# JiYuanFeng/DDP

Hardware: AMD Instinct MI355X
Metric: images/s at K DDIM steps (512x1024, 150-class) per GPU and whole node (higher is better)
Workload: dtype f32 (bf16x3-split MFMA products, fp32 accumulate); 1 GPU; ade_swin_t_k3_8x512x1024 (ADE20K Swin-T DDP decode head, 3-step DDIM, batch 8x512x1024 per GPU; x (8,256,128,256), random-init weights); images_per_call=8, ddim_steps=3, parallelism=dp1 (independent images, weights broadcast once), gemm_engine=bf16x3

## Files before the change

ddp_amd/_lib.py:

```python
import ctypes as C
import os

from . import build as _build

MAX_LAYERS = 12
MAX_STEPS = 64
ABI_VERSION = 6

TASK_SEG, TASK_DEPTH, TASK_BEV = 0, 1, 2
SAMPLER_DDIM, SAMPLER_DDPM = 0, 1
GEMM_F32_MFMA, GEMM_BF16X3 = 0, 1
FLAG_UNFUSED_LAYER, FLAG_UNFUSED_PROLOGUE, FLAG_RECORD_X0, FLAG_GATHER_GUESS_ZERO, FLAG_FCN_PREPARED, FLAG_FORCE_X0, FLAG_UNFUSED_TAIL, FLAG_SB_HEAD = 1, 2, 4, 8, 16, 32, 64, 128
FLAG_DEPTH_SCALE_UP, FLAG_DEPTH_NO_EPS = 256, 512
DEPTH_NORM_LINEAR, DEPTH_NORM_SOFTMAX, DEPTH_NORM_SIGMOID = 0, 1, 2
MAX_DEPTH_BINS = 256
NECK_WEIGHTS_READY = 1

_fp = C.c_void_p


class DdpCfg(C.Structure):
    _fields_ = [
        ('abi_version', C.c_int32), ('task', C.c_int32), ('sampler', C.c_int32), ('batch', C.c_int32),
        ('randsteps', C.c_int32), ('timesteps', C.c_int32), ('num_layers', C.c_int32),
# ... 3 lines not shown
        ('threshold', C.c_float),
        ('bev_in_min', C.c_float * 2), ('bev_in_max', C.c_float * 2),
        ('bev_out_first', C.c_float * 2), ('bev_out_step', C.c_float * 2),
        ('gemm_mode', C.c_int32), ('flags', C.c_int32),
        ('depth_n_bins', C.c_int32), ('depth_norm', C.c_int32), ('head_min_depth', C.c_float), ('head_max_depth', C.c_float),
    ]


LAYER_FIELDS = ['sampling_offsets_w', 'sampling_offsets_b', 'attention_weights_w', 'attention_weights_b',
                'value_proj_w', 'value_proj_b', 'output_proj_w', 'output_proj_b', 'ffn0_w', 'ffn0_b',
                'ffn1_w', 'ffn1_b', 'norm0_w', 'norm0_b', 'norm1_w', 'norm1_b', 'time_w', 'time_b']


class DdpLayerWeights(C.Structure):
    _fields_ = [(n, _fp) for n in LAYER_FIELDS]


TOP_FIELDS = ['transform_w', 'transform_b', 'time_freq', 'time1_w', 'time1_b', 'time3_w', 'time3_b',
              'embedding', 'head_w', 'head_b']


class DdpWeights(C.Structure):
    _fields_ = [(n, _fp) for n in TOP_FIELDS] + [('layers', DdpLayerWeights * MAX_LAYERS), ('depth_bins', _fp)]


class DdpStep(C.Structure):
    _fields_ = [('time_in', C.c_float), ('alpha', C.c_float), ('sigma', C.c_float),
                ('alpha_next', C.c_float), ('sigma_next', C.c_float), ('ddpm_c', C.c_float),
                ('ddpm_std', C.c_float), ('ddpm_add_noise', C.c_int32)]


class DdpFpnLevel(C.Structure):
    _fields_ = [('lat_w', _fp), ('lat_gn_w', _fp), ('lat_gn_b', _fp), ('out_w', _fp), ('out_gn_w', _fp), ('out_gn_b', _fp),
                ('in_channels', C.c_int), ('h', C.c_int), ('w', C.c_int)]


class DdpFcnConv(C.Structure):
    _fields_ = [('conv_w', _fp), ('conv_b', _fp), ('bn_w', _fp), ('bn_b', _fp), ('bn_mean', _fp), ('bn_var', _fp),
                ('bn_eps', C.c_float), ('time_w', _fp), ('time_b', _fp)]


class DdpSegAug(C.Structure):
    _fields_ = [('d_scores', _fp), ('h', C.c_int32), ('w', C.c_int32), ('img_h', C.c_int32), ('img_w', C.c_int32),
                ('crop_h', C.c_int32), ('crop_w', C.c_int32), ('flip', C.c_int32)]


class DdpDepthAug(C.Structure):
    _fields_ = [('d_depth', _fp), ('h', C.c_int32), ('w', C.c_int32), ('flip', C.c_int32)]


MAX_AUGS = 16
MAX_WINDOWS = 64

EXPORTS = ['ddp_last_error', 'ddp_abi_version', 'ddp_query_workspace', 'ddp_query_const_workspace', 'ddp_prepare',
           'ddp_prepare_geometry', 'ddp_sample', 'ddp_msda_forward_lds_workspace', 'ddp_msda_forward_lds', 'ddp_seg_aug_postprocess', 'ddp_seg_slide_postprocess', 'ddp_depth_postprocess',
           'ddp_x0_trace', 'ddp_head_forward', 'ddp_msda_forward', 'ddp_linear', 'ddp_linear_b3_workspace', 'ddp_linear_b3', 'ddp_time_embed', 'ddp_ddim_update_seg',
           'ddp_seg_x0_project', 'ddp_seg_postprocess', 'ddp_neck_msm_workspace', 'ddp_neck_msm', 'ddp_fcn_head_workspace', 'ddp_fcn_head_forward', 'ddp_sample_fcn_workspace', 'ddp_prepare_fcn', 'ddp_sample_fcn', 'ddp_neck_fpn_workspace', 'ddp_neck_fpn', 'ddp_neck_fpn_msm_workspace', 'ddp_neck_fpn_msm', 'ddp_profile_begin', 'ddp_profile_end', 'ddp_profile_read']

_libs = {}


class DdpError(RuntimeError):
    pass


def lib_path():
    return os.environ.get('DDP_LIB_PATH') or _build.LIB_PATH


def load(path=None):
    path = os.path.abspath(path or lib_path())
    if path in _libs:
        return _libs[path]
    if not os.path.exists(path):
        raise DdpError(f'{path} not found: build it with `python -m ddp_amd.build` '
                       '(hipcc --offload-arch=gfx950); ddp_amd has no non-HIP fallback')
    if path == os.path.abspath(_build.LIB_PATH) and _build.built_hash() != _build.source_hash():
        raise DdpError(f'{path} is stale: built from sources {_build.built_hash() or "<no stamp>"}, the tree holds '
                       f'{_build.source_hash()}; rebuild with `python -m ddp_amd.build`')
    lib = C.CDLL(path)
    lib.ddp_last_error.restype = C.c_char_p
    lib.ddp_abi_version.restype = C.c_int
    lib.ddp_query_workspace.argtypes = [C.POINTER(DdpCfg), C.POINTER(C.c_size_t)]
    lib.ddp_prepare.argtypes = [C.POINTER(DdpCfg), C.POINTER(DdpWeights), C.POINTER(DdpStep), _fp, _fp]
    lib.ddp_query_const_workspace.argtypes = [C.POINTER(DdpCfg), C.POINTER(C.c_size_t)]
    lib.ddp_prepare_geometry.argtypes = [C.POINTER(DdpCfg), _fp, _fp]
    lib.ddp_msda_forward_lds_workspace.argtypes = [C.c_int, C.c_int, C.c_int, C.POINTER(C.c_size_t)]
    lib.ddp_msda_forward_lds.argtypes = [_fp, _fp, _fp, _fp, C.c_int, C.c_int, C.c_int, _fp, _fp]
    lib.ddp_seg_aug_postprocess.argtypes = [C.POINTER(DdpSegAug), C.c_int, C.c_int, C.c_int, C.c_int, C.c_int, C.c_int, _fp, _fp,
                                            _fp]
    lib.ddp_seg_slide_postprocess.argtypes = [C.POINTER(_fp), C.POINTER(C.c_int), C.POINTER(C.c_int)] + [C.c_int] * 17 + [_fp, _fp, _fp]
    lib.ddp_depth_postprocess.argtypes = [C.POINTER(DdpDepthAug), C.c_int, C.c_int, C.c_int, C.c_int, C.c_int, C.c_float, C.c_float,
                                          _fp, _fp]
    lib.ddp_sample.argtypes = [C.POINTER(DdpCfg), C.POINTER(DdpWeights), C.POINTER(DdpStep), _fp, _fp, _fp, _fp,
                               _fp, _fp]
    lib.ddp_x0_trace.argtypes = [C.POINTER(DdpCfg), _fp, C.POINTER(C.c_void_p)]
    lib.ddp_head_forward.argtypes = [C.POINTER(DdpCfg), C.POINTER(DdpWeights), _fp, _fp, _fp, _fp, _fp]
    lib.ddp_msda_forward.argtypes = [_fp, _fp, _fp, C.c_int, C.c_int, C.c_int, _fp]
    lib.ddp_linear.argtypes = [_fp, _fp, _fp, _fp, C.c_int, C.c_int, C.c_int, C.c_int, _fp]
    lib.ddp_linear_b3_workspace.argtypes = [C.c_int, C.c_int, C.c_int, C.POINTER(C.c_size_t)]
    lib.ddp_linear_b3.argtypes = [_fp, _fp, _fp, _fp, C.c_int, C.c_int, C.c_int, _fp, _fp]
    lib.ddp_time_embed.argtypes = [C.POINTER(DdpWeights), C.c_int, C.POINTER(C.c_float), C.c_int, _fp, _fp, _fp, _fp]
    lib.ddp_ddim_update_seg.argtypes = [_fp, C.c_int, C.c_int, _fp, _fp, C.c_int, C.POINTER(DdpStep), _fp]
    lib.ddp_seg_x0_project.argtypes = [_fp, C.c_int, C.c_int, C.c_int, _fp, C.c_float, _fp, _fp]
    lib.ddp_seg_postprocess.argtypes = [_fp] + [C.c_int] * 12 + [_fp, _fp]
    lib.ddp_neck_msm_workspace.argtypes = [C.c_int, C.POINTER(C.c_int), C.POINTER(C.c_int), C.POINTER(C.c_size_t)]
    lib.ddp_neck_msm.argtypes = [C.POINTER(_fp), C.POINTER(C.c_int), C.POINTER(C.c_int), C.c_int, _fp, _fp, _fp, C.c_int, C.c_int, _fp,
# ... 30 lines not shown
```

ddp_amd/csrc/ddp_api.hip:

```cpp
#include <stdarg.h>
#include <stdio.h>
#include <string.h>

#include <initializer_list>

#include "ddp_internal.h"

namespace ddp {

static thread_local char g_err[512] = "";

void set_error(const char* fmt, ...) {
  va_list ap;
  va_start(ap, fmt);
  vsnprintf(g_err, sizeof(g_err), fmt, ap);
  va_end(ap);
}

int check_launch(const char* what) {
  hipError_t e = hipGetLastError();
  if (e != hipSuccess) {
    set_error("%s: %s", what, hipGetErrorString(e));
    return DDP_E_LAUNCH;
  }
// ... 456 lines not shown
      return DDP_E_LAUNCH;
    }
    DDP_TRY(launch_pack_conv3x3_scaled(w->head_w, nullptr, o.bins_wpack, o.nbins, 256, st));
    if (o.b3) {
      DDP_TRY(launch_split_weights(o.bins_wpack, 2304, 256, 2304, o.bins_wsplit, st));
      DDP_TRY(launch_build_stages(o.bins_wsplit, size_t(256) * 2304, 2304, 256, 0, 1, 72, 0, 2, 1, 0, o.bins_stream, st));
    }
  }
  for (int l = 0; l < o.L; ++l) {
    const ddp_layer_weights& lw = w->layers[l];
    DDP_TRY(launch_pack_rows(lw.sampling_offsets_w, 64, lw.attention_weights_w, 32, o.wcat[l], 256, st));
    DDP_TRY(launch_pack_rows(lw.sampling_offsets_b, 64, lw.attention_weights_b, 32, o.bcat[l], 1, st));
  }
  if (o.b3) {
    auto wr = [](const SplitW& w) { return const_cast<unsigned short*>(w.p); };
    DDP_TRY(launch_split_weights(o.wx, o.Cx, 256, o.Cx, wr(o.wp_x), st));
    if (c->task != DDP_TASK_DEPTH) DDP_TRY(launch_split_weights(o.wm, 256, 256, 256, wr(o.wp_m), st));
    if (c->task == DDP_TASK_DEPTH) DDP_TRY(launch_split_weights(o.wtap, 256, 9, 256, wr(o.wp_head), st));
    else DDP_TRY(launch_split_weights(w->head_w, 256, o.Kc, 256, wr(o.wp_head), st));
    for (int l = 0; l < o.L; ++l) {
      const ddp_layer_weights& lw = w->layers[l];
      DDP_TRY(launch_split_weights(lw.value_proj_w, 256, 256, 256, wr(o.wp_v[l]), st));
      DDP_TRY(launch_split_weights(o.wcat[l], 256, 96, 256, wr(o.wp_cat[l]), st));
      DDP_TRY(launch_split_weights(lw.output_proj_w, 256, 256, 256, wr(o.wp_o[l]), st));
      DDP_TRY(launch_split_weights(lw.ffn0_w, 256, DDP_FFN, 256, wr(o.wp_f0[l]), st));
      DDP_TRY(launch_split_weights(lw.ffn1_w, DDP_FFN, 256, DDP_FFN, wr(o.wp_f1[l]), st));
    }
    if (c->task == DDP_TASK_SEG) {
      const int nch = (o.Kc + 63) / 64;
      DDP_TRY(launch_build_stages(o.wp_head.p, o.wp_head.comp_stride, 256, o.Kc, 1, nch, 2, 0, 0, 1, 2, o.tail_stream, st));
      DDP_TRY(bias_table(o.tail_bias, {{0, w->head_b, o.Kc}}, "seg tail", st));
      DDP_TRY(launch_build_stages(o.wp_head.p, o.wp_head.comp_stride, 256, o.Kc, 1, nch, 2, 0, 0, 1, 2, o.tail4_stream, st));
      DDP_TRY(build_proj_images(o, 0, o.tail4_stream, 2 * nch, st));
      DDP_TRY(bias_table(o.tail4_bias, {{0, w->head_b, o.Kc}, {DDP_FFN, w->layers[0].value_proj_b, 256}}, "fused tail", st));
      DDP_TRY(launch_linear(o.lut, 256, false, o.wm, 256, nullptr, nullptr, 0, 0, 0, o.tlut, 256, o.Kc + 1, 256, 256, 0, st));
    }
    if (c->task != DDP_TASK_DEPTH)
      DDP_TRY(launch_build_stages(o.wp_m.p, o.wp_m.comp_stride, 256, 256, 0, 1, 8, 0, 2, 1, 0, o.pro_stream, st));
    DDP_TRY(build_proj_images(o, 0, o.pro_stream, 8, st));
    DDP_TRY(bias_table(o.pro_bias, {{DDP_FFN, w->layers[0].value_proj_b, 256}}, "prologue", st));
    if (o.head7_stream) {
      DDP_TRY(launch_build_stages(o.wp_m.p, o.wp_m.comp_stride, 256, 256, 0, 1, 8, 0, 2, 1, 0, o.head7_stream, st));
      DDP_TRY(launch_build_stages(o.wp_x.p, o.wp_x.comp_stride, 256, 256, 0, 1, 8, 8, 2, 1, 0, o.head7_stream, st));
      if (hipMemcpyAsync(o.head7_stream + size_t(16) * 48 * 1024, o.pro_stream + size_t(8) * 48 * 1024, size_t(11) * 48 * 1024,
                         hipMemcpyDeviceToDevice, st) != hipSuccess) {
        set_error("first-step head stream copy failed");
        return DDP_E_LAUNCH;
      }
    }
    for (int l = 0; l < o.L; ++l) {
      const ddp_layer_weights& lw = w->layers[l];
      unsigned char* sp = o.wstream[l];
      DDP_TRY(launch_build_stages(o.wp_o[l].p, o.wp_o[l].comp_stride, 256, 256, 0, 1, 8, 0, 2, 1, 0, sp, st));
      DDP_TRY(launch_build_stages(o.wp_f0[l].p, o.wp_f0[l].comp_stride, 256, DDP_FFN, 1, 16, 2, 8, 0, 1, 4, sp, st));
      DDP_TRY(launch_build_stages(o.wp_f1[l].p, o.wp_f1[l].comp_stride, DDP_FFN, 256, 0, 1, 32, 10, 4, 1, 0, sp, st));
      DDP_TRY(bias_table(o.bias_ext[l], {{0, lw.ffn0_b, DDP_FFN}}, "layer", st));
      if (l + 1 < o.L) {
        DDP_TRY(build_proj_images(o, l + 1, sp, 72, st));
        if (hipMemcpyAsync(o.bias_ext[l] + DDP_FFN, w->layers[l + 1].value_proj_b, 256 * sizeof(float), hipMemcpyDeviceToDevice, st) !=
            hipSuccess) {
          set_error("bias table copy failed");
          return DDP_E_LAUNCH;
        }
      }
    }
    if (o.lt_stream && c->task != DDP_TASK_SEG) {
      const size_t sb = size_t(48) * 1024;
      const int rows = c->task == DDP_TASK_DEPTH ? 9 : o.Kc;
      DDP_TRY(launch_build_stages(o.wp_head.p, o.wp_head.comp_stride, 256, rows, 1, 1, 2, 0, 0, 1, 2, o.tail_stream, st));
      DDP_TRY(bias_table(o.tail_bias, {{0, c->task == DDP_TASK_BEV ? w->head_b : nullptr, o.Kc}}, "head tail", st));
      if (hipMemcpyAsync(o.lt_stream, o.wstream[o.L - 1], 72 * sb, hipMemcpyDeviceToDevice, st) != hipSuccess ||
          hipMemcpyAsync(o.lt_stream + 72 * sb, o.tail_stream, 2 * sb, hipMemcpyDeviceToDevice, st) != hipSuccess) {
        set_error("layer + tail stream copy failed");
        return DDP_E_LAUNCH;
      }
      DDP_TRY(bias_table(o.lt_bias, {{0, w->layers[o.L - 1].ffn0_b, DDP_FFN}}, "layer + tail", st));
    }
    if (o.wvs) {
      DDP_TRY(launch_matvec(w->layers[0].value_proj_w, nullptr, o.wm, o.wvs, 256, 256, 1, 256, 256, 0, 0, st));
      DDP_TRY(launch_matvec(o.wcat[0], nullptr, o.wm, o.wvs + 256, 256, 96, 1, 256, 96, 0, 0, st));
    }
    if (o.lut64) {
      DDP_TRY(launch_build_bev_lut(w->embedding, o.lut64, o.Kc, c->bit_scale, st));
      DDP_TRY(launch_linear(o.lut64, 256, false, o.wm, 256, nullptr, nullptr, 0, 0, 0, o.tlut, 256, 1 << o.Kc, 256, 256, 0, st));
    }
    if (o.lt_stream && c->task == DDP_TASK_SEG) {
      const int nch = (o.Kc + 63) / 64;
      const size_t sb = size_t(48) * 1024;
      if (hipMemcpyAsync(o.lt_stream, o.wstream[o.L - 1], 72 * sb, hipMemcpyDeviceToDevice, st) != hipSuccess ||
          hipMemcpyAsync(o.lt_stream + 72 * sb, o.tail4_stream, size_t(2 * nch + 11) * sb, hipMemcpyDeviceToDevice, st) != hipSuccess) {
        set_error("layer + tail stream copy failed");
        return DDP_E_LAUNCH;
      }
      DDP_TRY(bias_table(o.lt_bias, {{0, w->layers[o.L - 1].ffn0_b, DDP_FFN}, {DDP_FFN, w->layers[0].value_proj_b, 256}}, "layer + tail",
                         st));
    }
  }
  return DDP_OK;
}

int publish_q(const Layout& o, const float* row_major, hipStream_t st) {
  if (o.b3 && !o.fused_layer) return launch_row_to_sb(row_major, 256, o.q_sb, int(o.M), 256, st);
  return launch_row_to_blk(row_major, o.q, int(o.M), st);
}

int depth_bins_head(const ddp_cfg* c, const Layout& o, float* pred, hipStream_t st) {
  const int M = int(o.M);
  DepthBinsArgs a;
// ... 417 lines not shown
    DDP_TRY(launch_bev_resample(o.xproj, o.s, o.B, geom, st));
    DDP_TRY(launch_nchw_to_sb(d_noise, o.in_sb, o.R, 256, o.N, st));
    DDP_TRY(launch_b3_linear(o.in_sb, o.wp_m, nullptr, nullptr, 0, 0, 0, o.feat0, 256, M0, 256, 256, st, TAG_FEAT));
  } else {
    DDP_TRY(launch_nchw_to_tok(d_noise, o.mask, o.R, 256, o.N, st));
  }
  TailLaunch tl{};
  tl.Q = o.q;
  tl.M = int(o.M);
  tl.num_classes = o.Kc;
  tl.kind = 1;
  tl.prob = o.prob;
  tl.threshold = c->threshold;
  tl.x0_idx = code;
  tl.ldl = 32;
  for (int s = 0; s < o.K; ++s) {
    const ddp_step& sp = steps[s];
    const float* aff = o.aff + size_t(s) * o.L * 512;
    if (p.bev_chain) {
      if (s > 0) {
        const ddp_step& pp = steps[s - 1];
        const float ua = pp.sigma_next / (pp.sigma > 1e-8f ? pp.sigma : 1e-8f);
        DDP_TRY(launch_bev_u_update(o.feat0, code, o.tlut, o.R, geom, ua, pp.alpha_next - pp.alpha * ua, st));
      }
      DDP_TRY(launch_bev_q(o.feat0, o.s, o.q, o.R, o.r, geom, st));
    } else {
      if (o.b3) {
        DDP_TRY(launch_row_to_sb(o.mask, 256, o.in_sb, M0, 256, st));
        DDP_TRY(launch_b3_linear(o.in_sb, o.wp_m, nullptr, o.xproj, 256, o.r * o.N, o.N, o.feat0, 256, M0, 256, 256, st, TAG_XPROJ));
      } else {
        DDP_TRY(launch_linear(o.mask, 256, false, o.wm, 256, nullptr, o.xproj, 256, o.r * o.N, o.N, o.feat0, 256, M0, 256, 256, 0, st));
      }
      DDP_TRY(launch_bev_resample(o.feat0, o.s, o.R, geom, st));
      DDP_TRY(publish_q(o, o.s, st));
    }
    tl.prob_mode = s == 0 ? 1 : 2;
    DDP_TRY(encoder_forward(w, o, aff, st, false, !p.bev_chain, p.bev_chain ? &tl : nullptr));
    if (p.bev_chain) continue;
    DDP_TRY(head_gemm(c, w, o, st));
    DDP_TRY(launch_bev_update(bev_update_args(c, w, o, o.mask, s == 0, sp), st));
  }
  return launch_finalize_nchw(o.prob, 32, d_out, o.B, o.r, o.Nh, o.Kc, float(o.r * o.K), st);
}

}
}

using namespace ddp;

extern "C" {

const char* ddp_last_error(void) { return g_err; }
int ddp_abi_version(void) { return DDP_ABI_VERSION; }

int ddp_profile_begin(int tag) {
  if ((tag < 0 || tag >= TAG_COUNT) && tag != PROF_ALL) {
    set_error("profile: unknown tag %d", tag);
    return DDP_E_BADCFG;
  }
  if (!g_prof.created) {
    for (int i = 0; i < 2 * PROF_MAX; ++i)
      if (hipEventCreate(&g_prof.ev[i]) != hipSuccess) {
        set_error("hipEventCreate failed");
        return DDP_E_LAUNCH;
      }
    g_prof.created = true;
  }
  g_prof.n = 0;
  g_prof.tag = tag;
  g_prof.resolved = false;
  return DDP_OK;
}

int ddp_profile_end(float* total_ms, int* launches) {
  const int n = g_prof.n;
  g_prof.tag = -1;
  float tot = 0.f;
  for (int i = 0; i < n; ++i) {
    if (hipEventSynchronize(g_prof.ev[2 * i + 1]) != hipSuccess) {
      set_error("hipEventSynchronize failed");
      return DDP_E_LAUNCH;
    }
    float ms = 0.f;
    (void)hipEventElapsedTime(&ms, g_prof.ev[2 * i], g_prof.ev[2 * i + 1]);
    g_prof.ms[i] = ms;
    tot += ms;
  }
  g_prof.resolved = true;
  if (total_ms) *total_ms = tot;
  if (launches) *launches = n;
  return DDP_OK;
}

int ddp_profile_read(int tag, float* total_ms, int* launches) {
  if (tag < 0 || tag >= TAG_COUNT) {
    set_error("profile: unknown tag %d", tag);
    return DDP_E_BADCFG;
  }
  if (!g_prof.resolved) {
    set_error("profile: no finished session (call ddp_profile_end first)");
    return DDP_E_BADCFG;
  }
  float tot = 0.f;
  int cnt = 0;
  for (int i = 0; i < g_prof.n; ++i)
    if (g_prof.rec_tag[i] == tag) {
// ... 1093 lines not shown
```

ddp_amd/csrc/ddp_internal.h:

```cpp
#pragma once
#include <hip/hip_runtime.h>
#include <stddef.h>
#include <atomic>
#include "../../include/ddp_mi355x.h"


#ifndef DDP_S_F32
#define DDP_S_F32 1
#endif

namespace ddp {

void set_error(const char* fmt, ...);
int check_launch(const char* what);

struct LdsAttrOnce {
  std::atomic<unsigned long long> done{0};
  void ensure(const void* fn, int bytes) {
    int dev = 0;
    (void)hipGetDevice(&dev);
    if (dev >= 0 && dev < 64 && ((done.load(std::memory_order_acquire) >> dev) & 1ull)) return;
    if (hipFuncSetAttribute(fn, hipFuncAttributeMaxDynamicSharedMemorySize, bytes) != hipSuccess) {
      (void)hipGetLastError();
      set_error("hipFuncSetAttribute(MaxDynamicSharedMemorySize = %d) failed on device %d", bytes, dev);
// ... 1 lines not shown
    }
    if (dev >= 0 && dev < 64) done.fetch_or(1ull << dev, std::memory_order_release);
  }
};
inline int cu_count() {
  static std::atomic<int> cache[64];
  int dev = 0;
  (void)hipGetDevice(&dev);
  if (dev >= 0 && dev < 64) {
    const int c = cache[dev].load(std::memory_order_relaxed);
    if (c > 0) return c;
  }
  int n = 0;
  if (hipDeviceGetAttribute(&n, hipDeviceAttributeMultiprocessorCount, dev) != hipSuccess || n <= 0) n = 256;
  if (dev >= 0 && dev < 64) cache[dev].store(n, std::memory_order_relaxed);
  return n;
}

enum GemmTag {
  TAG_GENERIC = 0, TAG_XPROJ = 1, TAG_FEAT = 2, TAG_VALUE = 3, TAG_SAMP = 4, TAG_OUTPROJ_LN = 5, TAG_FC1 = 6,
  TAG_FC2_LN = 7, TAG_HEAD = 8, TAG_GATHER = 9, TAG_LAYER_TAIL = 10, TAG_COUNT = 11
};
void prof_begin(int tag, hipStream_t st);
void prof_end(int tag, hipStream_t st);

int launch_linear(const float* A, int lda, bool a_blk, const float* W, int ldw, const float* bias, const float* add,
                  int ld_add, int rn, int n_tok, float* out, int ldo, int M, int N, int K, int gelu, hipStream_t st,
                  int tag = TAG_GENERIC);
int launch_linear_blk(const float* A, int lda, bool a_blk, const float* W, int ldw, const float* bias,
                      const float* add, int ld_add, int rn, int n_tok, float* out_blk, int M, int N, int K, int gelu,
                      hipStream_t st);
int launch_linear_res_ln_blk(const float* A, int lda, bool a_blk, const float* W, int ldw, const float* bias,
                             const float* res_blk, const float* ga_aff, const float* be_aff, float* out_blk, int M,
                             int K, hipStream_t st);
int launch_linear_samp(const float* A_blk, const float* Wcat, const float* py, const float* px, int n_tok, int w,
                       float* out, int M, hipStream_t st);

struct SplitW {
  const unsigned short* p;
  size_t comp_stride;
};
int launch_b3_linear(const unsigned short* A_sb, const SplitW& w, const float* bias, const float* add, int ld_add,
                     int rn, int n_tok, float* out, int ldo, int M, int N, int K, hipStream_t st, int tag);
int launch_b3_linear_sb(const unsigned short* A_sb, const SplitW& w, const float* bias, const float* add, int ld_add,
                        int rn, int n_tok, unsigned short* out_sb, float* out_f32_blk, int M, int N, int K, int gelu,
                        hipStream_t st, int tag);
int launch_b3_linear_res_ln(const unsigned short* A_sb, const SplitW& w, const float* bias, const float* res_blk,
                            const unsigned short* res_sb, const float* ga_aff, const float* be_aff, float* out_f32_blk,
                            unsigned short* out_sb, int M, int K, hipStream_t st, int tag);
int launch_b3_linear_samp(const unsigned short* A_sb, const SplitW& wcat, const float* py, const float* px, int n_tok,
                          int w, float* out, int M, hipStream_t st);
int launch_build_stages(const unsigned short* Wp, size_t comp_stride, int K, int rows_valid, int tall, int n_rowblk, int n_kblk,
                        int base, int a, int b, int c, unsigned char* stream, hipStream_t st);
struct LayerLaunch {
  const unsigned short* S;
  const float* Sf;
  float* Q;
  unsigned short* Q_sb;
  const unsigned char* stream;
  const float* bias_ext;
  const float *bo, *ga0, *be0, *b2, *ga1, *be1;
  int M, has_next;
  float* v_out;
  float* samp_out;
  const float *py, *px;
  int n_tok, w;
  const float* res_f;
  const float* wm;
  const float* dvec;
};
int launch_b3_layer(const LayerLaunch& a, hipStream_t st);
struct TailLaunch {
  float* Q;
  const unsigned char* stream;
  const float* bias_ext;
  const float* lut;
  float* prob;
  unsigned short* mask_sb;
  unsigned char* x0_idx;
  const unsigned char* x0_force;
  int M, num_classes, ldl, prob_mode;
  float alpha, sigma, alpha_next, sigma_next;
  int fuse_next;
  float* ubuf;
  const float* tlut;
  const float* res;
  int res_rn;
  int res_frag;
  float* v_out;
  float* samp_out;
  const float *py, *px;
  int n_tok, w;
  int kind;
  float threshold;
};
int launch_b3_tail(const TailLaunch& a, hipStream_t st);
bool b3_layer_tail_supported(int num_classes);
int launch_b3_layer_tail(const LayerLaunch& l, const TailLaunch& t, const unsigned char* stream, const float* bias_ext,
                         const float* seg_bias, hipStream_t st);
struct PrologueLaunch {
  const unsigned short* mask_sb;
  float* Q;
  const unsigned char* stream;
  const float* bias_ext;
  const float* res;
  int res_rn;
// ... 180 lines not shown
```

ddp_amd/csrc/layer_bf16x3.h:

```cpp
#pragma once
#include <type_traits>

#include "gemm_bf16x3.h"

namespace ddp {
namespace b3 {

constexpr int LYR_BM = 128;
constexpr int LYR_THREADS = 256;
constexpr int LYR_STAGE_B = 48 * 1024;
constexpr int LYR_RING = 3;
constexpr int LYR_BIAS_OFF = LYR_RING * LYR_STAGE_B;
constexpr int LYR_BIAS_N = 1024 + 256 + 128;
constexpr int LYR_T_BO = LYR_BIAS_N, LYR_T_GA0 = LYR_T_BO + 256, LYR_T_BE0 = LYR_T_GA0 + 256, LYR_T_B2 = LYR_T_BE0 + 256,
              LYR_T_GA1 = LYR_T_B2 + 256, LYR_T_BE1 = LYR_T_GA1 + 256,
              LYR_T_SEG = LYR_T_BE1 + 256,
              LYR_TABLE_N = LYR_T_SEG + 256;
static_assert(LYR_T_SEG % 64 == 0, "bias_init addresses the table in chunks of 64 floats");
constexpr size_t LYR_LDS_B = size_t(LYR_BIAS_OFF) + LYR_TABLE_N * 4;
constexpr int LYR_ST_OUT = 8, LYR_ST_FFN = 64, LYR_ST_NEXT = 11;
constexpr int LYR_STAGES = LYR_ST_OUT + LYR_ST_FFN + LYR_ST_NEXT;

struct LayerArgs {
  const unsigned short* S;
// ... 1021 lines not shown
        }
    }

    DDP_LYR_STAMP_AT(0)
    {
      float sum = 0.f;
#pragma unroll
      for (int t = 0; t < 8; ++t)
#pragma unroll
        for (int r = 0; r < 16; ++r) {
          const float v = acc2[t][r] + qr[t][r >> 2][r & 3];
          acc2[t][r] = v;
          sum += v;
        }
      const float mean = half_sum(sum) * (1.0f / 256.0f);
      float var = 0.f;
#pragma unroll
      for (int t = 0; t < 8; ++t)
#pragma unroll
        for (int r = 0; r < 16; ++r) {
          const float d = acc2[t][r] - mean;
          acc2[t][r] = d;
          var += d * d;
        }
      const float rstd = 1.0f / sqrtf(half_sum(var) * (1.0f / 256.0f) + 1e-5f);
#pragma unroll
      for (int t = 0; t < 8; ++t) {
#pragma unroll
        for (int g = 0; g < 4; ++g) {
          const int ch = t * 32 + 8 * g + 4 * ht;
          const f32x4 ga = *reinterpret_cast<const f32x4*>(bias_s + LYR_T_GA0 + ch);
          const f32x4 be = *reinterpret_cast<const f32x4*>(bias_s + LYR_T_BE0 + ch);
#pragma unroll
          for (int e = 0; e < 4; ++e) acc2[t][4 * g + e] = acc2[t][4 * g + e] * (rstd * ga[e]) + be[e];
        }
#pragma unroll
        for (int gp = 0; gp < 2; ++gp) {
          float xv[8];
#pragma unroll
          for (int e = 0; e < 8; ++e) xv[e] = acc2[t][8 * gp + e];
          split8_packed(xv, xa[2 * t + gp][0], xa[2 * t + gp][1], xa[2 * t + gp][2]);
        }
#pragma unroll
        for (int g = 0; g < 4; ++g) {
          const f32x4 b = *reinterpret_cast<const f32x4*>(bias_s + LYR_T_B2 + t * 32 + 8 * g + 4 * ht);
#pragma unroll
          for (int e = 0; e < 4; ++e) acc2[t][4 * g + e] += b[e];
        }
      }
    }

    DDP_LYR_STAMP_AT(1)
    refresh();
    for (int hc = 0; hc < 16; ++hc) {
      f32x16 acc1[2];
      bias_init(acc1, hc);
      tall_pair(acc1[0], acc1[1], I0);
      DDP_LYR_STAMP_AT(2)
      u32x4 hcur[3], hn[3];
      {
        float xg[8];
#pragma unroll
        for (int e = 0; e < 8; ++e) xg[e] = acc1[0][e];
        gelu_split8_packed(xg, hcur[0], hcur[1], hcur[2]);
      }
      DDP_LYR_STAMP_AT(3)
      u32x4 w[2][3];
#pragma unroll
      for (int t = 0; t < 2; ++t)
#pragma unroll
        for (int c = 0; c < 3; ++c) w[t][c] = frag2(slot, c, t, 0);
#pragma unroll
      for (int s2 = 0; s2 < 2; ++s2) {
        stage_begin(nxt(nxt(slot)));
        const int nslot = nxt(slot);
#pragma unroll
        for (int ks = 0; ks < 2; ++ks) {
          const int kb = s2 * 2 + ks;
          const int kn = kb + 1;
#pragma unroll
          for (int tpp = 0; tpp < 2; ++tpp) {
            GeluState g0, g1, g2, g3;
            const float v0 = kb < 3 ? acc1[kn >> 1][8 * (kn & 1) + 4 * tpp] : 0.f;
            const float v1 = kb < 3 ? acc1[kn >> 1][8 * (kn & 1) + 4 * tpp + 1] : 0.f;
            const float v2 = kb < 3 ? acc1[kn >> 1][8 * (kn & 1) + 4 * tpp + 2] : 0.f;
            const float v3 = kb < 3 ? acc1[kn >> 1][8 * (kn & 1) + 4 * tpp + 3] : 0.f;
            auto block = [&](auto halfc) __attribute__((always_inline)) {
              constexpr int half = decltype(halfc)::value;
              const int tp = 2 * tpp + half;
              const int blk = ks * 4 + tp;
              const bool hand = s2 == 0 && blk == 7;
              const bool nb = blk + 1 < 8 || hand;
              const int rs = hand ? nslot : slot;
              const int tp2 = hand ? 0 : (tp + 1 < 4 ? tp + 1 : 0), ks2 = hand ? 0 : (tp + 1 < 4 ? ks : ks + 1);
              if (hand) {
                __builtin_amdgcn_s_waitcnt(0x0F7B);
                __syncthreads();
              }
              auto fill = [&](auto kc) __attribute__((always_inline)) {
                constexpr int k = decltype(kc)::value;
                if (k == 0 && nb) w[0][2] = frag2(rs, 2, 2 * tp2, ks2);
                if (k == 1 && nb) w[1][2] = frag2(rs, 2, 2 * tp2 + 1, ks2);
                if (k == 4 && nb) w[0][1] = frag2(rs, 1, 2 * tp2, ks2);
                if (k == 5 && nb) w[1][1] = frag2(rs, 1, 2 * tp2 + 1, ks2);
                if (k == 10 && nb) w[0][0] = frag2(rs, 0, 2 * tp2, ks2);
                if (k == 11 && nb) w[1][0] = frag2(rs, 0, 2 * tp2 + 1, ks2);
                if (k == 3) dma(blk, blk + 1);
                if (k == 8 && blk < 4) dma(8 + blk, 9 + blk);
                if (kb < 3) {
                  constexpr int sl = half * 12 + k;
                  gelu_maybe<GELU_SCHED[sl][0]>(g0, v0);
                  gelu_maybe<GELU_SCHED[sl][1]>(g1, v1);
                  gelu_maybe<GELU_SCHED[sl][2]>(g2, v2);
                  gelu_maybe<GELU_SCHED[sl][3]>(g3, v3);
                  if (sl == 21) {
                    hn[0][2 * tpp] = __builtin_amdgcn_perm(gelu_ph(g1), gelu_ph(g0), 0x07060302);
                    hn[0][2 * tpp + 1] = __builtin_amdgcn_perm(gelu_ph(g3), gelu_ph(g2), 0x07060302);
                  }
                  if (sl == 22) {
                    hn[1][2 * tpp] = __builtin_amdgcn_perm(gelu_pm(g1), gelu_pm(g0), 0x07060302);
                    hn[1][2 * tpp + 1] = __builtin_amdgcn_perm(gelu_pm(g3), gelu_pm(g2), 0x07060302);
                  }
                  if (sl == 23) {
                    hn[2][2 * tpp] = __builtin_amdgcn_perm(gelu_pl(g1), gelu_pl(g0), 0x07060302);
                    hn[2][2 * tpp + 1] = __builtin_amdgcn_perm(gelu_pl(g3), gelu_pl(g2), 0x07060302);
                  }
                }
              };
              DDP_LYR_BLOCK(acc2[2 * tp], acc2[2 * tp + 1], hcur[0], hcur[1], hcur[2], fill)
            };
            block(I0);
            block(I1);
          }
          if (kb < 3) {
#pragma unroll
            for (int c = 0; c < 3; ++c) hcur[c] = hn[c];
          }
        }
        if (s2 == 1) {
          wait_vm12();
          __syncthreads();
        }
        slot = nxt(slot);
      }
      DDP_LYR_STAMP_AT(4)
    }

    refresh();
    {
      float* qst = la.Q + grp * 8192 + lane * 4;
      asm volatile("" : "+v"(qst));
      char* qsb = reinterpret_cast<char*>(la.Q_sb) + grp * 256 * 192 + lane * 16;
      f32x2 sum2 = {0.f, 0.f};
#pragma unroll
      for (int t = 0; t < 8; ++t)
#pragma unroll
        for (int r = 0; r < 16; r += 2) sum2 += f32x2{acc2[t][r], acc2[t][r + 1]};
      const float mean = half_sum(sum2[0] + sum2[1]) * (1.0f / 256.0f);
      const f32x2 mean2 = {mean, mean};
      f32x2 var2 = {0.f, 0.f};
#pragma unroll
      for (int t = 0; t < 8; ++t)
#pragma unroll
        for (int r = 0; r < 16; r += 2) {
          const f32x2 d = f32x2{acc2[t][r], acc2[t][r + 1]} - mean2;
          acc2[t][r] = d[0];
          acc2[t][r + 1] = d[1];
          var2 = __builtin_elementwise_fma(d, d, var2);
        }
      const float rstd = 1.0f / sqrtf(half_sum(var2[0] + var2[1]) * (1.0f / 256.0f) + 1e-5f);
      const f32x2 rstd2 = {rstd, rstd};
#pragma unroll
      for (int t = 0; t < 8; ++t) {
#pragma unroll
        for (int g = 0; g < 4; ++g) {
          const int ch = t * 32 + 8 * g + 4 * ht;
          const f32x4 ga = *reinterpret_cast<const f32x4*>(bias_s + LYR_T_GA1 + ch);
          const f32x4 be = *reinterpret_cast<const f32x4*>(bias_s + LYR_T_BE1 + ch);
#pragma unroll
          for (int e = 0; e < 4; e += 2) {
            const f32x2 y = __builtin_elementwise_fma(f32x2{acc2[t][4 * g + e], acc2[t][4 * g + e + 1]},
                                                     rstd2 * f32x2{ga[e], ga[e + 1]}, f32x2{be[e], be[e + 1]});
            acc2[t][4 * g + e] = y[0];
            acc2[t][4 * g + e + 1] = y[1];
          }
        }
#pragma unroll
        for (int gp = 0; gp < 2; ++gp) {
          const int b = 2 * t + gp;
          float xv[8];
#pragma unroll
          for (int e = 0; e < 8; ++e) xv[e] = acc2[t][8 * gp + e];
          split8_packed(xv, xa[b][0], xa[b][1], xa[b][2]);
          if constexpr (!LT) {
            store_q_block(qst, b, xv);
            if (la.Q_sb) {
// ... 333 lines not shown
```

include/ddp_mi355x.h:

```cpp
#ifndef DDP_MI355X_H
#define DDP_MI355X_H

#include <stddef.h>
#include <stdint.h>

#ifdef __cplusplus
extern "C" {
#endif
#if defined(__GNUC__)
#pragma GCC visibility push(default)
#endif

#define DDP_ABI_VERSION 6
#define DDP_MAX_LAYERS 12
#define DDP_MAX_STEPS 64
#define DDP_EMBED 256
#define DDP_HEADS 8
#define DDP_POINTS 4
#define DDP_FFN 1024
#define DDP_TIME_DIM 1024
#define DDP_SINU_FEATS 17
#define DDP_SAMP_STRIDE 96

enum { DDP_OK = 0, DDP_E_BADCFG = -1, DDP_E_ALIGN = -2, DDP_E_LAUNCH = -3, DDP_E_NULL = -4 };
// ... 13 lines not shown
typedef struct ddp_cfg {
  int32_t abi_version;
  int32_t task;
  int32_t sampler;
  int32_t batch;
  int32_t randsteps;
  int32_t timesteps;
  int32_t num_layers;
  int32_t num_classes;
  int32_t feat_channels;
  int32_t h, w;
  int32_t head_h, head_w;
  int32_t accumulation;
  float bit_scale;
  float min_depth, max_depth;
  float threshold;
  float bev_in_min[2], bev_in_max[2], bev_out_first[2], bev_out_step[2];
  int32_t gemm_mode;
  int32_t flags;
  int32_t depth_n_bins;
  int32_t depth_norm;
  float head_min_depth, head_max_depth;
} ddp_cfg;

typedef struct ddp_layer_weights {
  const float *sampling_offsets_w, *sampling_offsets_b;
  const float *attention_weights_w, *attention_weights_b;
  const float *value_proj_w, *value_proj_b;
  const float *output_proj_w, *output_proj_b;
  const float *ffn0_w, *ffn0_b;
  const float *ffn1_w, *ffn1_b;
  const float *norm0_w, *norm0_b, *norm1_w, *norm1_b;
  const float *time_w, *time_b;
} ddp_layer_weights;

typedef struct ddp_weights {
  const float *transform_w, *transform_b;
  const float *time_freq;
  const float *time1_w, *time1_b;
  const float *time3_w, *time3_b;
  const float *embedding;
  const float *head_w, *head_b;
  ddp_layer_weights layers[DDP_MAX_LAYERS];
  const float* depth_bins;
} ddp_weights;

typedef struct ddp_step {
  float time_in, alpha, sigma, alpha_next, sigma_next, ddpm_c, ddpm_std;
  int32_t ddpm_add_noise;
} ddp_step;

const char* ddp_last_error(void);
int ddp_abi_version(void);

int ddp_query_workspace(const ddp_cfg* cfg, size_t* bytes);

int ddp_prepare(const ddp_cfg* cfg, const ddp_weights* weights, const ddp_step* steps,
                void* d_workspace, void* stream);

int ddp_query_const_workspace(const ddp_cfg* cfg, size_t* bytes);
int ddp_prepare_geometry(const ddp_cfg* cfg, void* d_workspace, void* stream);

int ddp_sample(const ddp_cfg* cfg, const ddp_weights* weights, const ddp_step* steps,
               const float* d_x, const float* d_noise, const float* d_step_noise, float* d_out,
               void* d_workspace, void* stream);

int ddp_x0_trace(const ddp_cfg* cfg, void* d_workspace, const unsigned char** d_idx);


int ddp_head_forward(const ddp_cfg* cfg, const ddp_weights* weights, const float* d_feat,
                     const float* d_temb, float* d_out, void* d_workspace, void* stream);

int ddp_msda_forward(const float* d_value, const float* d_samp, float* d_out, int rows, int h, int w,
                     void* stream);

int ddp_msda_forward_lds_workspace(int rows, int h, int w, size_t* bytes);
int ddp_msda_forward_lds(const float* d_value, const float* d_samp, const float* d_guess, float* d_out, int rows, int h, int w,
                         void* d_workspace, void* stream);

int ddp_linear(const float* d_a, const float* d_w, const float* d_bias, float* d_out, int m, int n, int k,
               int gelu, void* stream);

int ddp_linear_b3_workspace(int m, int n, int k, size_t* bytes);
int ddp_linear_b3(const float* d_a, const float* d_w, const float* d_bias, float* d_out, int m, int n, int k,
                  void* d_workspace, void* stream);

int ddp_time_embed(const ddp_weights* weights, int num_layers, const float* time_in_host, int s,
                   float* d_temb, float* d_film, float* d_scratch , void* stream);

int ddp_ddim_update_seg(const float* d_logits, int ld_logits, int num_classes, const float* d_lut,
                        float* d_mask, int rows, const ddp_step* step, void* stream);

int ddp_seg_x0_project(const float* d_scores, int batch, int num_classes, int n_pix, const float* d_embedding,
                       float bit_scale, float* d_x0, void* stream);

int ddp_seg_postprocess(const float* d_scores, int batch, int num_classes, int h, int w, int img_h, int img_w,
                        int crop_h, int crop_w, int out_h, int out_w, int align_corners, int flip,
                        unsigned char* d_seg, void* stream);

#define DDP_MAX_AUGS 16
typedef struct ddp_seg_aug {
  const float* d_scores;
  int32_t h, w;
  int32_t img_h, img_w;
  int32_t crop_h, crop_w;
  int32_t flip;
// ... 77 lines not shown
```

Measured before the change: 257.5 images/s.

## Interleave FFN fc1 and fc2 chunk GEMMs with staggered GELU in bf16x3 layer

Restructures the fused FFN loop so that the fc1 GEMM plus GELU for chunk hc+1 is software-pipelined against the fc2 GEMM for chunk hc. Weight stage images are rebuilt per 64-wide chunk with interleaved slot ordering so that fc1 and fc2 stages alternate in the stream. The aim is to hide the GELU and the serial fc1 tail latency behind MFMA work and to keep the DMA stream continuous. In exchange it adds register pressure (px and hk buffers) and more complex slot bookkeeping.

```diff
diff --git a/ddp_amd/_lib.py b/ddp_amd/_lib.py
--- a/ddp_amd/_lib.py
+++ b/ddp_amd/_lib.py
@@ -79,7 +79,7 @@
 MAX_AUGS = 16
 MAX_WINDOWS = 64
 
-EXPORTS = ['ddp_last_error', 'ddp_abi_version', 'ddp_query_workspace', 'ddp_query_const_workspace', 'ddp_prepare',
+EXPORTS = ['ddp_last_error', 'ddp_abi_version', 'ddp_ffn_stage_slot', 'ddp_query_workspace', 'ddp_query_const_workspace', 'ddp_prepare',
            'ddp_prepare_geometry', 'ddp_sample', 'ddp_msda_forward_lds_workspace', 'ddp_msda_forward_lds', 'ddp_seg_aug_postprocess', 'ddp_seg_slide_postprocess', 'ddp_depth_postprocess',
            'ddp_x0_trace', 'ddp_head_forward', 'ddp_msda_forward', 'ddp_linear', 'ddp_linear_b3_workspace', 'ddp_linear_b3', 'ddp_time_embed', 'ddp_ddim_update_seg',
            'ddp_seg_x0_project', 'ddp_seg_postprocess', 'ddp_neck_msm_workspace', 'ddp_neck_msm', 'ddp_fcn_head_workspace', 'ddp_fcn_head_forward', 'ddp_sample_fcn_workspace', 'ddp_prepare_fcn', 'ddp_sample_fcn', 'ddp_neck_fpn_workspace', 'ddp_neck_fpn', 'ddp_neck_fpn_msm_workspace', 'ddp_neck_fpn_msm', 'ddp_profile_begin', 'ddp_profile_end', 'ddp_profile_read']
diff --git a/ddp_amd/csrc/ddp_api.hip b/ddp_amd/csrc/ddp_api.hip
--- a/ddp_amd/csrc/ddp_api.hip
+++ b/ddp_amd/csrc/ddp_api.hip
@@ -532,8 +532,12 @@
       const ddp_layer_weights& lw = w->layers[l];
       unsigned char* sp = o.wstream[l];
       DDP_TRY(launch_build_stages(o.wp_o[l].p, o.wp_o[l].comp_stride, 256, 256, 0, 1, 8, 0, 2, 1, 0, sp, st));
-      DDP_TRY(launch_build_stages(o.wp_f0[l].p, o.wp_f0[l].comp_stride, 256, DDP_FFN, 1, 16, 2, 8, 0, 1, 4, sp, st));
-      DDP_TRY(launch_build_stages(o.wp_f1[l].p, o.wp_f1[l].comp_stride, DDP_FFN, 256, 0, 1, 32, 10, 4, 1, 0, sp, st));
+      for (int ch = 0; ch < DDP_FFN / 64; ++ch) {
+        DDP_TRY(launch_build_stages(o.wp_f0[l].p + size_t(ch) * 64 * 256, o.wp_f0[l].comp_stride, 256, 64, 1, 1, 2,
+                                    ffn_stage_slot(0, ch), 0, 1, 0, sp, st));
+        DDP_TRY(launch_build_stages(o.wp_f1[l].p + size_t(ch) * 64, o.wp_f1[l].comp_stride, DDP_FFN, 256, 0, 1, 2,
+                                    ffn_stage_slot(1, ch), 0, 1, 0, sp, st));
+      }
       DDP_TRY(bias_table(o.bias_ext[l], {{0, lw.ffn0_b, DDP_FFN}}, "layer", st));
       if (l + 1 < o.L) {
         DDP_TRY(build_proj_images(o, l + 1, sp, 72, st));
@@ -1057,6 +1061,7 @@
 
 const char* ddp_last_error(void) { return g_err; }
 int ddp_abi_version(void) { return DDP_ABI_VERSION; }
+int ddp_ffn_stage_slot(int fc2, int chunk) { return (chunk < 0 || chunk >= DDP_FFN / 64) ? -1 : ffn_stage_slot(fc2 != 0, chunk); }
 
 int ddp_profile_begin(int tag) {
   if ((tag < 0 || tag >= TAG_COUNT) && tag != PROF_ALL) {
diff --git a/ddp_amd/csrc/ddp_internal.h b/ddp_amd/csrc/ddp_internal.h
--- a/ddp_amd/csrc/ddp_internal.h
+++ b/ddp_amd/csrc/ddp_internal.h
@@ -77,6 +77,10 @@
                           int w, float* out, int M, hipStream_t st);
 int launch_build_stages(const unsigned short* Wp, size_t comp_stride, int K, int rows_valid, int tall, int n_rowblk, int n_kblk,
                         int base, int a, int b, int c, unsigned char* stream, hipStream_t st);
+inline int ffn_stage_slot(int fc2, int c) {
+  const int pair = fc2 ? (c < 15 ? 2 * c + 2 : 31) : (c == 0 ? 0 : 2 * c - 1);
+  return 8 + 2 * pair;
+}
 struct LayerLaunch {
   const unsigned short* S;
   const float* Sf;
diff --git a/ddp_amd/csrc/layer_bf16x3.h b/ddp_amd/csrc/layer_bf16x3.h
--- a/ddp_amd/csrc/layer_bf16x3.h
+++ b/ddp_amd/csrc/layer_bf16x3.h
@@ -1097,96 +1097,185 @@
 
     DDP_LYR_STAMP_AT(1)
     refresh();
-    for (int hc = 0; hc < 16; ++hc) {
-      f32x16 acc1[2];
-      bias_init(acc1, hc);
-      tall_pair(acc1[0], acc1[1], I0);
-      DDP_LYR_STAMP_AT(2)
-      u32x4 hcur[3], hn[3];
-      {
-        float xg[8];
-#pragma unroll
-        for (int e = 0; e < 8; ++e) xg[e] = acc1[0][e];
-        gelu_split8_packed(xg, hcur[0], hcur[1], hcur[2]);
-      }
-      DDP_LYR_STAMP_AT(3)
-      u32x4 w[2][3];
-#pragma unroll
-      for (int t = 0; t < 2; ++t)
-#pragma unroll
-        for (int c = 0; c < 3; ++c) w[t][c] = frag2(slot, c, t, 0);
-#pragma unroll
-      for (int s2 = 0; s2 < 2; ++s2) {
-        stage_begin(nxt(nxt(slot)));
-        const int nslot = nxt(slot);
-#pragma unroll
-        for (int ks = 0; ks < 2; ++ks) {
-          const int kb = s2 * 2 + ks;
-          const int kn = kb + 1;
-#pragma unroll
-          for (int tpp = 0; tpp < 2; ++tpp) {
-            GeluState g0, g1, g2, g3;
-            const float v0 = kb < 3 ? acc1[kn >> 1][8 * (kn & 1) + 4 * tpp] : 0.f;
-            const float v1 = kb < 3 ? acc1[kn >> 1][8 * (kn & 1) + 4 * tpp + 1] : 0.f;
-            const float v2 = kb < 3 ? acc1[kn >> 1][8 * (kn & 1) + 4 * tpp + 2] : 0.f;
-            const float v3 = kb < 3 ? acc1[kn >> 1][8 * (kn & 1) + 4 * tpp + 3] : 0.f;
+    {
+      float px[32];
+      u32x4 hk[4][3];
+      auto ffn_fc2 = [&](auto steadyc, f32x16 (&a1)[2]) __attribute__((always_inline)) {
+        constexpr bool STEADY = decltype(steadyc)::value != 0;
+        u32x4 w[2][3];
+#pragma unroll
+        for (int t = 0; t < 2; ++t)
+#pragma unroll
+          for (int c = 0; c < 3; ++c) w[t][c] = frag2(slot, c, t, 0);
+#pragma unroll
+        for (int s2 = 0; s2 < 2; ++s2) {
+          stage_begin(nxt(nxt(slot)));
+          const int nslot = nxt(slot);
+#pragma unroll
+          for (int ks = 0; ks < 2; ++ks) {
+            const int kb = s2 * 2 + ks;
+#pragma unroll
+            for (int tpp = 0; tpp < 2; ++tpp) {
+              const int bp = 2 * kb + tpp;
+              const bool dense = STEADY ? kb == 2 : kb < 3;
+              const bool light = STEADY && kb < 2;
+              const bool move = STEADY && kb == 3;
+              const int kn = kb < 3 ? kb + 1 : 3;
+              const int vi = dense ? 8 * kn + 4 * tpp : light ? 16 + 2 * bp : 0;
+              GeluState g0, g1, g2, g3;
+              const float v0 = px[vi], v1 = px[vi + 1], v2 = px[vi + 2], v3 = px[vi + 3];
+              auto block = [&](auto halfc) __attribute__((always_inline)) {
+                constexpr int half = decltype(halfc)::value;
+                const int tp = 2 * tpp + half;
+                const int blk = ks * 4 + tp;
+                const bool hand = s2 == 0 && blk == 7;
+                const bool nb = blk + 1 < 8 || hand;
+                const int rs = hand ? nslot : slot;
+                const int tp2 = hand ? 0 : (tp + 1 < 4 ? tp + 1 : 0), ks2 = hand ? 0 : (tp + 1 < 4 ? ks : ks + 1);
+                if (hand) {
+                  __builtin_amdgcn_s_waitcnt(0x0F7B);
+                  __syncthreads();
+                }
+                auto fill = [&](auto kc) __attribute__((always_inline)) {
+                  constexpr int k = decltype(kc)::value;
+                  if (k == 0 && nb) w[0][2] = frag2(rs, 2, 2 * tp2, ks2);
+                  if (k == 1 && nb) w[1][2] = frag2(rs, 2, 2 * tp2 + 1, ks2);
+                  if (k == 4 && nb) w[0][1] = frag2(rs, 1, 2 * tp2, ks2);
+                  if (k == 5 && nb) w[1][1] = frag2(rs, 1, 2 * tp2 + 1, ks2);
+                  if (k == 10 && nb) w[0][0] = frag2(rs, 0, 2 * tp2, ks2);
+                  if (k == 11 && nb) w[1][0] = frag2(rs, 0, 2 * tp2 + 1, ks2);
+                  if (k == 3) dma(blk, blk + 1);
+                  if (k == 8 && blk < 4) dma(8 + blk, 9 + blk);
+                  constexpr int sl = half * 12 + k;
+                  if (dense || light) {
+                    gelu_maybe<GELU_SCHED[sl][0]>(g0, v0);
+                    gelu_maybe<GELU_SCHED[sl][1]>(g1, v1);
+                  }
+                  if (dense) {
+                    gelu_maybe<GELU_SCHED[sl][2]>(g2, v2);
+                    gelu_maybe<GELU_SCHED[sl][3]>(g3, v3);
+                    if (sl == 21) {
+                      hk[kn][0][2 * tpp] = __builtin_amdgcn_perm(gelu_ph(g1), gelu_ph(g0), 0x07060302);
+                      hk[kn][0][2 * tpp + 1] = __builtin_amdgcn_perm(gelu_ph(g3), gelu_ph(g2), 0x07060302);
+                    }
+                    if (sl == 22) {
+                      hk[kn][1][2 * tpp] = __builtin_amdgcn_perm(gelu_pm(g1), gelu_pm(g0), 0x07060302);
+                      hk[kn][1][2 * tpp + 1] = __builtin_amdgcn_perm(gelu_pm(g3), gelu_pm(g2), 0x07060302);
+                    }
+                    if (sl == 23) {
+                      hk[kn][2][2 * tpp] = __builtin_amdgcn_perm(gelu_pl(g1), gelu_pl(g0), 0x07060302);
+                      hk[kn][2][2 * tpp + 1] = __builtin_amdgcn_perm(gelu_pl(g3), gelu_pl(g2), 0x07060302);
+                    }
+                  }
+                  if (light) {
+                    if (sl == 21) hk[2][0][bp & 3] = __builtin_amdgcn_perm(gelu_ph(g1), gelu_ph(g0), 0x07060302);
+                    if (sl == 22) hk[2][1][bp & 3] = __builtin_amdgcn_perm(gelu_pm(g1), gelu_pm(g0), 0x07060302);
+                    if (sl == 23) hk[2][2][bp & 3] = __builtin_amdgcn_perm(gelu_pl(g1), gelu_pl(g0), 0x07060302);
+                  }
+                  if (move) {
+                    constexpr int m0 = k == 2 ? 0 : k == 3 ? 1 : k == 6 ? 2 : k == 7 ? 4 : k == 8 ? 6 : k == 9 ? 7 : -1;
+                    constexpr int mn = (k == 6 || k == 7) ? 2 : 1;
+                    if constexpr (m0 >= 0) {
+                      const int pb = 8 * (2 * tpp + half);
+#pragma unroll
+                      for (int i = m0; i < m0 + mn; ++i) px[pb + i] = a1[(pb + i) >> 4][(pb + i) & 15];
+                    }
+                  }
+                };
+                DDP_LYR_BLOCK(acc2[2 * tp], acc2[2 * tp + 1], hk[kb][0], hk[kb][1], hk[kb][2], fill)
+              };
+              block(I0);
+              block(I1);
+            }
+          }
+          if (s2 == 1) {
+            wait_vm12();
+            __syncthreads();
+          }
+          slot = nxt(slot);
+        }
+      };
+      auto ffn_fc1_gelu = [&](f32x16& a0, f32x16& a1) __attribute__((always_inline)) {
+        u32x4 w[2][3];
+#pragma unroll
+        for (int t = 0; t < 2; ++t)
+#pragma unroll
+          for (int c = 0; c < 3; ++c) w[t][c] = frag1(slot, c, t, 0);
+#pragma unroll
+        for (int s1 = 0; s1 < 2; ++s1) {
+          stage_begin(nxt(nxt(slot)));
+          const int nslot = nxt(slot);
+#pragma unroll
+          for (int bq = 0; bq < 4; ++bq) {
+            const int bp = 4 * s1 + bq;
+            GeluState g0, g1;
+            const float v0 = px[2 * bp], v1 = px[2 * bp + 1];
             auto block = [&](auto halfc) __attribute__((always_inline)) {
               constexpr int half = decltype(halfc)::value;
-              const int tp = 2 * tpp + half;
-              const int blk = ks * 4 + tp;
-              const bool hand = s2 == 0 && blk == 7;
-              const bool nb = blk + 1 < 8 || hand;
-              const int rs = hand ? nslot : slot;
-              const int tp2 = hand ? 0 : (tp + 1 < 4 ? tp + 1 : 0), ks2 = hand ? 0 : (tp + 1 < 4 ? ks : ks + 1);
+              const int b = 2 * bq + half;
+              const bool nb = b + 1 < 8;
+              const bool hand = s1 == 0 && b == 7;
+              const int rs = hand ? nslot : slot, rb = hand ? 0 : b + 1;
+              const int kb = s1 * 8 + b;
               if (hand) {
-                __builtin_amdgcn_s_waitcnt(0x0F7B);
+                wait_hand(false);
                 __syncthreads();
               }
               auto fill = [&](auto kc) __attribute__((always_inline)) {
                 constexpr int k = decltype(kc)::value;
-                if (k == 0 && nb) w[0][2] = frag2(rs, 2, 2 * tp2, ks2);
-                if (k == 1 && nb) w[1][2] = frag2(rs, 2, 2 * tp2 + 1, ks2);
-                if (k == 4 && nb) w[0][1] = frag2(rs, 1, 2 * tp2, ks2);
-                if (k == 5 && nb) w[1][1] = frag2(rs, 1, 2 * tp2 + 1, ks2);
-                if (k == 10 && nb) w[0][0] = frag2(rs, 0, 2 * tp2, ks2);
-                if (k == 11 && nb) w[1][0] = frag2(rs, 0, 2 * tp2 + 1, ks2);
-                if (k == 3) dma(blk, blk + 1);
-                if (k == 8 && blk < 4) dma(8 + blk, 9 + blk);
-                if (kb < 3) {
-                  constexpr int sl = half * 12 + k;
-                  gelu_maybe<GELU_SCHED[sl][0]>(g0, v0);
-                  gelu_maybe<GELU_SCHED[sl][1]>(g1, v1);
-                  gelu_maybe<GELU_SCHED[sl][2]>(g2, v2);
-                  gelu_maybe<GELU_SCHED[sl][3]>(g3, v3);
-                  if (sl == 21) {
-                    hn[0][2 * tpp] = __builtin_amdgcn_perm(gelu_ph(g1), gelu_ph(g0), 0x07060302);
-                    hn[0][2 * tpp + 1] = __builtin_amdgcn_perm(gelu_ph(g3), gelu_ph(g2), 0x07060302);
-                  }
-                  if (sl == 22) {
-                    hn[1][2 * tpp] = __builtin_amdgcn_perm(gelu_pm(g1), gelu_pm(g0), 0x07060302);
-                    hn[1][2 * tpp + 1] = __builtin_amdgcn_perm(gelu_pm(g3), gelu_pm(g2), 0x07060302);
-                  }
-                  if (sl == 23) {
-                    hn[2][2 * tpp] = __builtin_amdgcn_perm(gelu_pl(g1), gelu_pl(g0), 0x07060302);
-                    hn[2][2 * tpp + 1] = __builtin_amdgcn_perm(gelu_pl(g3), gelu_pl(g2), 0x07060302);
-                  }
-                }
+                if (k == 0 && (nb || hand)) w[0][2] = frag1(rs, 2, 0, rb);
+                if (k == 1 && (nb || hand)) w[1][2] = frag1(rs, 2, 1, rb);
+                if (k == 4 && (nb || hand)) w[0][1] = frag1(rs, 1, 0, rb);
+                if (k == 5 && (nb || hand)) w[1][1] = frag1(rs, 1, 1, rb);
+                if (k == 10 && (nb || hand)) w[0][0] = frag1(rs, 0, 0, rb);
+                if (k == 11 && (nb || hand)) w[1][0] = frag1(rs, 0, 1, rb);
+                dma_slot(false, b, k);
+                constexpr int sl = half * 12 + k;
+                gelu_maybe<GELU_SCHED[sl][0]>(g0, v0);
+                gelu_maybe<GELU_SCHED[sl][1]>(g1, v1);
+                if (sl == 21) hk[bp >> 2][0][bp & 3] = __builtin_amdgcn_perm(gelu_ph(g1), gelu_ph(g0), 0x07060302);
+                if (sl == 22) hk[bp >> 2][1][bp & 3] = __builtin_amdgcn_perm(gelu_pm(g1), gelu_pm(g0), 0x07060302);
+                if (sl == 23) hk[bp >> 2][2][bp & 3] = __builtin_amdgcn_perm(gelu_pl(g1), gelu_pl(g0), 0x07060302);
               };
-              DDP_LYR_BLOCK(acc2[2 * tp], acc2[2 * tp + 1], hcur[0], hcur[1], hcur[2], fill)
+              DDP_LYR_BLOCK(a0, a1, xa[kb][0], xa[kb][1], xa[kb][2], fill)
             };
             block(I0);
             block(I1);
           }
-          if (kb < 3) {
-#pragma unroll
-            for (int c = 0; c < 3; ++c) hcur[c] = hn[c];
-          }
-        }
-        if (s2 == 1) {
-          wait_vm12();
-          __syncthreads();
-        }
-        slot = nxt(slot);
+          if (s1 == 1) {
+            wait_vm12();
+            __syncthreads();
+          }
+          slot = nxt(slot);
+        }
+      };
+
+      {
+        f32x16 acc1[2];
+        bias_init(acc1, 0);
+        tall_pair(acc1[0], acc1[1], I0);
+#pragma unroll
+        for (int i = 0; i < 32; ++i) px[i] = acc1[i >> 4][i & 15];
+      }
+      DDP_LYR_STAMP_AT(2)
+      for (int hc = 0; hc < 15; ++hc) {
+        f32x16 acc1[2];
+        bias_init(acc1, hc + 1);
+        ffn_fc1_gelu(acc1[0], acc1[1]);
+        DDP_LYR_STAMP_AT(2)
+        ffn_fc2(I1, acc1);
+        DDP_LYR_STAMP_AT(4)
+      }
+      {
+        float xg[8];
+#pragma unroll
+        for (int e = 0; e < 8; ++e) xg[e] = px[e];
+        gelu_split8_packed(xg, hk[0][0], hk[0][1], hk[0][2]);
+      }
+      DDP_LYR_STAMP_AT(3)
+      {
+        f32x16 none[2];
+        ffn_fc2(I0, none);
       }
       DDP_LYR_STAMP_AT(4)
     }
diff --git a/include/ddp_mi355x.h b/include/ddp_mi355x.h
--- a/include/ddp_mi355x.h
+++ b/include/ddp_mi355x.h
@@ -89,6 +89,7 @@
 
 const char* ddp_last_error(void);
 int ddp_abi_version(void);
+int ddp_ffn_stage_slot(int fc2, int chunk);
 
 int ddp_query_workspace(const ddp_cfg* cfg, size_t* bytes);
 
```

Measured after the change: 259.3 images/s (median of 6 runs). About the same (+0.7%).
